# SqueezeAILab/KVQuant

Hardware: NVIDIA H100
Metric: decode tokens/sec @ seqlen 128K (LLaMA-7B, bs1) (higher is better)
Workload: dtype f32

## Files before the change

kvquant_b200/csrc/kvq_kscore.cu:

```cuda
#include "kvq_kscore.cuh"
#include <cuda_fp16.h>
#include <stdlib.h>

namespace kvq {

template <int BITS> struct KCfg {
  static constexpr int N = 1 << BITS;
  static constexpr int W = Layout<BITS>::kWords;
  static constexpr int G = (BITS == 2) ? 16 : 128 / N;
  static constexpr int kThreads = 512;
  static constexpr int TT = kThreads;
  static constexpr int NRW = (BITS == 3) ? 4 : 2;
  static constexpr int D = (BITS == 4) ? 8 : 4;
};

__device__ __forceinline__ void cp_async4(uint32_t smem_dst, const void* gsrc, uint64_t pol, int pred) {
  asm volatile("{ .reg .pred p; setp.ne.s32 p, %3, 0;"
               " @p cp.async.ca.shared.global.L2::cache_hint [%0], [%1], 4, %2; }"
               ::"r"(smem_dst), "l"(gsrc), "l"(pol), "r"(pred) : "memory");
}
__device__ __forceinline__ void cp_async_commit() { asm volatile("cp.async.commit_group;" ::: "memory"); }
template <int N> __device__ __forceinline__ void cp_async_wait() { asm volatile("cp.async.wait_group %0;" ::"n"(N) : "memory"); }
__device__ __forceinline__ uint32_t lds_u32(uint32_t addr) {
  uint32_t v;
  asm volatile("ld.shared.u32 %0, [%1];" : "=r"(v) : "r"(addr));
  return v;
}

template <int BITS> __device__ __forceinline__ int chunk_word_row(int a, int i) {
  if constexpr (BITS == 4) { return i == 0 ? a : a + 8; }
  else if constexpr (BITS == 2) { return i == 0 ? (a >> 1) : 4 + (a >> 1); }
  else {
    const int first = (24 * (a & 3)) >> 5;
    const int w = (i & 1) ? min(first + 1, 2) : first;
    return 3 * ((a >> 2) + ((i >> 1) ? 2 : 0)) + w;
  }
}

template <int BITS>
__device__ __forceinline__ void k_item(const uint32_t* __restrict__ w, const int a, const uint32_t base,
                                       const float2* __restrict__ cs, float2& acc) {
  constexpr int N = 1 << BITS;
  constexpr int HI = kHalf * N * 8;
  if constexpr (BITS == 4) {
    const uint32_t e0 = (w[0] << 3) & 0x78787878u, o0 = (w[0] >> 1) & 0x78787878u;
    const uint32_t e1 = (w[1] << 3) & 0x78787878u, o1 = (w[1] >> 1) & 0x78787878u;
    static_for<0, 8>([&](auto ik) {
      constexpr int k = decltype(ik)::v;
      ffma2(acc, cs[k], lds_f2<k * N * 8>(__byte_perm((k & 1) ? o0 : e0, base, 0x7650 | (k >> 1))));
      ffma2(acc, cs[k], lds_f2<k * N * 8 + HI>(__byte_perm((k & 1) ? o1 : e1, base, 0x7650 | (k >> 1))));
    });
  } else if constexpr (BITS == 2) {
    const int sh = 16 * (a & 1);
    const uint32_t x0 = w[0] >> sh, x1 = w[1] >> sh;
    const uint32_t m00 = (x0 << 3) & 0x1818u, m01 = (x0 << 1) & 0x1818u, m02 = (x0 >> 1) & 0x1818u, m03 = (x0 >> 3) & 0x1818u;
    const uint32_t m10 = (x1 << 3) & 0x1818u, m11 = (x1 << 1) & 0x1818u, m12 = (x1 >> 1) & 0x1818u, m13 = (x1 >> 3) & 0x1818u;
    static_for<0, 8>([&](auto ik) {
      constexpr int k = decltype(ik)::v;
      const uint32_t s0 = (k & 3) == 0 ? m00 : ((k & 3) == 1 ? m01 : ((k & 3) == 2 ? m02 : m03));
      const uint32_t s1 = (k & 3) == 0 ? m10 : ((k & 3) == 1 ? m11 : ((k & 3) == 2 ? m12 : m13));
      ffma2(acc, cs[k], lds_f2<k * N * 8>(__byte_perm(s0, base, 0x7650 | (k >> 2))));
      ffma2(acc, cs[k], lds_f2<k * N * 8 + HI>(__byte_perm(s1, base, 0x7650 | (k >> 2))));
    });
  } else {
    const int sh = (24 * (a & 3)) & 31;
    const uint32_t x0 = __funnelshift_r(w[0], w[1], sh), x1 = __funnelshift_r(w[2], w[3], sh);
    static_for<0, 8>([&](auto ik) {
      constexpr int k = decltype(ik)::v;
      const uint32_t a0 = ((k == 0 ? (x0 << 3) : (x0 >> (3 * k - 3))) & 0x38u) | base;
      const uint32_t a1 = ((k == 0 ? (x1 << 3) : (x1 >> (3 * k - 3))) & 0x38u) | base;
      ffma2(acc, cs[k], lds_f2<k * N * 8>(a0));
      ffma2(acc, cs[k], lds_f2<k * N * 8 + HI>(a1));
    });
  }
}

template <int BITS, bool FULL>
__global__ void __launch_bounds__(KCfg<BITS>::kThreads, 1) k_scores_kernel(const KParams p) {
  using C = KCfg<BITS>;
  constexpr int N = C::N, W = C::W, G = C::G, TT = C::TT, NRW = C::NRW;
  constexpr int PD = (BITS == 4) ? 8 : 4;
  extern __shared__ unsigned char smem_raw[];
  unsigned char* smem = smem_raw + ((256u - (smem_u32(smem_raw) & 255u)) & 255u);
  float2* s_tab = reinterpret_cast<float2*>(smem);
  float* s_q = reinterpret_cast<float*>(s_tab + G * kHeadDim * N);

  const int tid = threadIdx.x;
  const uint64_t pol_stream = policy_evict_first(), pol_keep = policy_evict_last();
  const int h0 = blockIdx.y * G;
  const int nh = FULL ? G : min(G, p.H - h0);

  for (int i = tid; i < nh * kHeadDim; i += C::kThreads) s_q[i] = p.q[(int64_t)h0 * kHeadDim + i];
  __syncthreads();
  for (int i = tid; i < G * kHeadDim * N; i += C::kThreads) {
    float2 e = make_float2(0.f, 0.f);
    if (i < nh * kHeadDim * N) {
      const int hc = i / N;
      const int c = hc & (kHeadDim - 1);
      const float l = p.lut[((int64_t)h0 * kHeadDim) * N + i];
      const float qa = s_q[hc];
      const float qb = s_q[hc ^ kHalf];
      e = make_float2(l * qa, (c < kHalf) ? (l * qb) : -(l * qb));
    }
    s_tab[i] = e;
  }
  __syncthreads();
  const uint32_t tab0 = smem_u32(s_tab);

  const int64_t L_eff = k_eff_len(p);
  const int64_t range = k_eff_range(p, L_eff);
  const int64_t t_begin = (int64_t)blockIdx.x * range;
  const int64_t t_limit = min(L_eff, t_begin + range);
  if (t_begin >= t_limit) return;
  const uint32_t pitch = (uint32_t)p.Lmax * 4u;
  const unsigned char* cb0 = reinterpret_cast<const unsigned char*>(p.cache + (int64_t)h0 * W * p.Lmax);

  const unsigned char* src_cur = cb0 + (t_begin + tid) * 4;
  bool ok_cur = (t_begin + tid) < t_limit;

  uint32_t wq[PD][NRW];
#pragma unroll
  for (int d = 0; d < PD; ++d)
#pragma unroll
    for (int i = 0; i < NRW; ++i) wq[d][i] = 0;
  auto fetch = [&](uint32_t* dst, const unsigned char* base, bool ok, int a, int hl) {
    if (ok && (FULL || hl < nh)) {
#pragma unroll
      for (int i = 0; i < NRW; ++i)
        dst[i] = ld_stream_u32(reinterpret_cast<const uint32_t*>(
                                   base + (uint64_t)(uint32_t)(hl * W + chunk_word_row<BITS>(a, i)) * pitch), pol_stream);
    }
  };
  auto load_cs = [&](float2* dst, const int64_t t, int a) {
    if (t < t_limit) {
      const float2* rp = p.rope + (t + p.pos_offset) + (int64_t)(8 * a) * p.rope_npos;
#pragma unroll
      for (int k = 0; k < 8; ++k) dst[k] = ld_keep_f2(rp + (int64_t)k * p.rope_npos, pol_keep);
    }
  };

  static_for<0, PD>([&](auto id) { constexpr int d = decltype(id)::v; fetch(wq[d], src_cur, ok_cur, 0, d); });
  float2 cs[8], csn[8];
#pragma unroll
  for (int k = 0; k < 8; ++k) { cs[k] = make_float2(0.f, 0.f); csn[k] = make_float2(0.f, 0.f); }
  load_cs(cs, t_begin + tid, 0);

  for (int64_t tb = t_begin; tb < t_limit; tb += TT) {
    const int64_t t = tb + tid;
    const bool live = t < t_limit;
    const unsigned char* src_nxt = src_cur + TT * 4;
    const bool ok_nxt = (t + TT) < t_limit;
    if (tb + (tid & ~31) < t_limit) {
    float2 acc[G];
#pragma unroll
    for (int g = 0; g < G; ++g) acc[g] = make_float2(0.f, 0.f);

    for (int a = 0; a < 8; ++a) {
      load_cs(csn, a == 7 ? t + TT : t, (a + 1) & 7);
      const unsigned char* src_w = (a == 7) ? src_nxt : src_cur;
      const bool ok_w = (a == 7) ? ok_nxt : ok_cur;
      const int a_w = (a + 1) & 7;
      static_for<0, G>([&](auto ig) {
        constexpr int hl = decltype(ig)::v;
        uint32_t w[NRW];
#pragma unroll
        for (int i = 0; i < NRW; ++i) w[i] = wq[hl % PD][i];
        if constexpr (hl + PD < G) fetch(wq[hl % PD], src_cur, ok_cur, a, hl + PD);
        else fetch(wq[hl % PD], src_w, ok_w, a_w, hl + PD - G);
        k_item<BITS>(w, a, tab0 + (uint32_t)hl * (kHeadDim * N * 8) + (uint32_t)a * (8 * N * 8), cs, acc[hl]);
      });
#pragma unroll
      for (int k = 0; k < 8; ++k) cs[k] = csn[k];
    }

    float old[G];
#pragma unroll
    for (int hl = 0; hl < G; ++hl) {
      old[hl] = 0.f;
      if (p.accumulate && live && hl < nh) old[hl] = p.out[(int64_t)(h0 + hl) * p.out_stride + t];
    }
    if (p.opart != nullptr && live) {
      const float4* src = reinterpret_cast<const float4*>(p.opart + t * p.opart_stride + h0);
#pragma unroll
      for (int i = 0; i < G / 4; ++i) {
        const float4 v = __ldcg(src + i);
        old[4 * i] += v.x; old[4 * i + 1] += v.y; old[4 * i + 2] += v.z; old[4 * i + 3] += v.w;
      }
    }
#pragma unroll
    for (int hl = 0; hl < G; ++hl) {
      if (hl < nh) {
        const float s = ((acc[hl].x + acc[hl].y) + old[hl]) * p.scale;
        if (live) p.out[(int64_t)(h0 + hl) * p.out_stride + t] = s;
        if (p.gmax != nullptr) {
          const float m = warp_max(live ? s : -INFINITY);
          if ((tid & 31) == 0 && m > -INFINITY) atomic_max_float(p.gmax + h0 + hl, m);
        }
      }
    }
    }
    src_cur = src_nxt;
    ok_cur = ok_nxt;
  }
}

constexpr int kMaxConstHeads = 48;
__constant__ float4 c_qrot[kMaxConstHeads * kHalf];

template <int BITS> struct KKCfg {
  static constexpr int N = 1 << BITS;
  static constexpr int W = Layout<BITS>::kWords;
  static constexpr int CS = (N * 4 < 32) ? 32 : N * 4;
  static constexpr int G = (BITS == 4) ? 16 : 32;
  static constexpr int kThreads = 512;
  static constexpr int TT = kThreads;
  static constexpr int NRW = (BITS == 3) ? 4 : 2;
  static constexpr int D = 4;
};

template <int IMM>
__device__ __forceinline__ float lds_f1(uint32_t addr) {
  float v;
  asm("ld.shared.f32 %0, [%1+%2];" : "=f"(v) : "r"(addr), "n"(IMM));
  return v;
}
__device__ __forceinline__ float2 fmul2(const float2 a, const float2 b) {
  return make_float2(__fmul_rn(a.x, b.x), __fmul_rn(a.y, b.y));
}

template <int BITS>
__device__ __forceinline__ void kk_item(const uint32_t* __restrict__ w, const int a, const uint32_t base, const int hq,
                                        const float2* __restrict__ cs, float2& acc) {
  using C = KKCfg<BITS>;
  constexpr int CS = C::CS;
  constexpr int HI = kHalf * CS;
  uint32_t alo[8], ahi[8];
  if constexpr (BITS == 4) {
    const uint32_t e0 = (w[0] << 2) & 0x3C3C3C3Cu, o0 = (w[0] >> 2) & 0x3C3C3C3Cu;
    const uint32_t e1 = (w[1] << 2) & 0x3C3C3C3Cu, o1 = (w[1] >> 2) & 0x3C3C3C3Cu;
    static_for<0, 8>([&](auto ik) {
      constexpr int k = decltype(ik)::v;
      alo[k] = __byte_perm((k & 1) ? o0 : e0, base, 0x7650 | (k >> 1));
      ahi[k] = __byte_perm((k & 1) ? o1 : e1, base, 0x7650 | (k >> 1));
    });
  } else if constexpr (BITS == 2) {
    const int sh = 16 * (a & 1);
    const uint32_t x0 = w[0] >> sh, x1 = w[1] >> sh;
    const uint32_t m00 = (x0 << 2) & 0x0C0Cu, m01 = x0 & 0x0C0Cu, m02 = (x0 >> 2) & 0x0C0Cu, m03 = (x0 >> 4) & 0x0C0Cu;
    const uint32_t m10 = (x1 << 2) & 0x0C0Cu, m11 = x1 & 0x0C0Cu, m12 = (x1 >> 2) & 0x0C0Cu, m13 = (x1 >> 4) & 0x0C0Cu;
    static_for<0, 8>([&](auto ik) {
      constexpr int k = decltype(ik)::v;
      const uint32_t s0 = (k & 3) == 0 ? m00 : ((k & 3) == 1 ? m01 : ((k & 3) == 2 ? m02 : m03));
      const uint32_t s1 = (k & 3) == 0 ? m10 : ((k & 3) == 1 ? m11 : ((k & 3) == 2 ? m12 : m13));
      alo[k] = __byte_perm(s0, base, 0x7650 | (k >> 2));
      ahi[k] = __byte_perm(s1, base, 0x7650 | (k >> 2));
    });
  } else {
    const int sh = (24 * (a & 3)) & 31;
    const uint32_t x0 = __funnelshift_r(w[0], w[1], sh), x1 = __funnelshift_r(w[2], w[3], sh);
    static_for<0, 8>([&](auto ik) {
      constexpr int k = decltype(ik)::v;
      alo[k] = ((3 * k >= 2 ? (x0 >> (3 * k - 2)) : (x0 << (2 - 3 * k))) & 0x1Cu) | base;
      ahi[k] = ((3 * k >= 2 ? (x1 >> (3 * k - 2)) : (x1 << (2 - 3 * k))) & 0x1Cu) | base;
    });
  }
  static_for<0, 8>([&](auto ik) {
    constexpr int k = decltype(ik)::v;
    const float2 x = make_float2(lds_f1<k * CS>(alo[k]), lds_f1<k * CS + HI>(ahi[k]));
    const float4 qr = c_qrot[hq * kHalf + 8 * a + k];
    const float2 kap = [&] {
      const float2 t = fmul2(make_float2(cs[k].y, cs[k].y), make_float2(qr.z, qr.w));
      float2 r = t;
      ffma2(r, make_float2(cs[k].x, cs[k].x), make_float2(qr.x, qr.y));
      return r;
    }();
    ffma2(acc, x, kap);
  });
}

template <int BITS>
__global__ void __launch_bounds__(KKCfg<BITS>::kThreads, 1) k_scores_kappa_kernel(const KParams p) {
  using C = KKCfg<BITS>;
  constexpr int N = C::N, W = C::W, G = C::G, TT = C::TT, NRW = C::NRW, D = C::D, CS = C::CS;
  extern __shared__ unsigned char smem_raw[];
  unsigned char* smem = smem_raw + ((256u - (smem_u32(smem_raw) & 255u)) & 255u);
  unsigned char* s_tab = smem;
  uint32_t* s_ring = reinterpret_cast<uint32_t*>(smem + (size_t)G * kHeadDim * CS);

  const int tid = threadIdx.x;
  const uint64_t pol_stream = policy_evict_first(), pol_keep = policy_evict_last();
  const int h0 = blockIdx.y * G;
  const int nh = min(G, p.H - h0);

  for (int i = tid; i < nh * kHeadDim * N; i += C::kThreads) {
    const int hc = i / N, code = i - hc * N;
    *reinterpret_cast<float*>(s_tab + (size_t)hc * CS + code * 4) = p.lut[((int64_t)h0 * kHeadDim) * N + i];
  }
  __syncthreads();
  const uint32_t tab0 = smem_u32(s_tab);
  const uint32_t ring0 = smem_u32(s_ring) + tid * 4;

  const int64_t tile_first = (int64_t)blockIdx.x * p.tiles_per_cta;
  const int64_t tile_end = min(tile_first + p.tiles_per_cta, (p.L + TT - 1) / TT);
  const int64_t t_limit = min(p.L, tile_end * TT);
  const uint32_t* cbase = p.cache + (int64_t)h0 * W * p.Lmax;
  const uint32_t pitch = (uint32_t)p.Lmax * 4u;
  const unsigned char* cb0 = reinterpret_cast<const unsigned char*>(cbase);
  int64_t t_cur = tile_first * TT + tid;
  auto prefetch = [&](int nxt, int a, int hl, int slot) {
    const int64_t t = t_cur + (nxt ? TT : 0);
    const int ok = (t < t_limit) && (hl < nh);
    const unsigned char* src = cb0 + t * 4;
#pragma unroll
    for (int i = 0; i < NRW; ++i)
      cp_async4(ring0 + (uint32_t)(slot * NRW + i) * (TT * 4),
                src + (uint64_t)(uint32_t)(hl * W + chunk_word_row<BITS>(a, i)) * pitch, pol_stream, ok);
    cp_async_commit();
  };
  auto load_cs = [&](float2* dst, int64_t tile, int a) {
    const int64_t t = tile * TT + tid;
    if (t < t_limit) {
      const float2* rp = p.rope + (t + p.pos_offset) + (int64_t)(8 * a) * p.rope_npos;
#pragma unroll
      for (int k = 0; k < 8; ++k) dst[k] = ld_keep_f2(rp + (int64_t)k * p.rope_npos, pol_keep);
    }
  };

  static_for<0, D>([&](auto id) {
    constexpr int d = decltype(id)::v;
    prefetch((d / G) / 8, (d / G) % 8, d % G, d % D);
  });
  float2 cs[8], csn[8];
#pragma unroll
  for (int k = 0; k < 8; ++k) { cs[k] = make_float2(0.f, 0.f); csn[k] = make_float2(0.f, 0.f); }
  load_cs(cs, tile_first, 0);

  for (int64_t tile = tile_first; tile < tile_end; ++tile) {
    const int64_t t = tile * TT + tid;
    t_cur = t;
    const bool live = t < p.L;
    float2 acc[G];
#pragma unroll
    for (int g = 0; g < G; ++g) acc[g] = make_float2(0.f, 0.f);

    for (int a = 0; a < 8; ++a) {
      load_cs(csn, a == 7 ? tile + 1 : tile, (a + 1) & 7);
      static_for<0, G>([&](auto ig) {
        constexpr int hl = decltype(ig)::v;
        cp_async_wait<D - 1>();
        uint32_t w[NRW];
        constexpr int slot = hl % D;
#pragma unroll
        for (int i = 0; i < NRW; ++i) w[i] = lds_u32(ring0 + (uint32_t)(slot * NRW + i) * (TT * 4));
        {
          constexpr int hn = (hl + D) % G;
          constexpr int wrap = (hl + D) / G;
          const int an = a + wrap;
          prefetch(an >> 3, an & 7, hn, slot);
        }
        if (hl < nh)
          kk_item<BITS>(w, a, tab0 + (uint32_t)hl * (kHeadDim * CS) + (uint32_t)a * (8 * CS), h0 + hl, cs, acc[hl]);
      });
#pragma unroll
      for (int k = 0; k < 8; ++k) cs[k] = csn[k];
    }

#pragma unroll
    for (int hl = 0; hl < G; ++hl) {
      if (hl < nh) {
        float s = acc[hl].x + acc[hl].y;
        if (live) {
          float* o = p.out + (int64_t)(h0 + hl) * p.out_stride + t;
          if (p.accumulate) s += *o;
          s *= p.scale;
          *o = s;
        }
        if (p.gmax != nullptr) {
          const float m = warp_max(live ? s : -INFINITY);
          if ((tid & 31) == 0 && m > -INFINITY) atomic_max_float(p.gmax + h0 + hl, m);
        }
      }
    }
  }
  cp_async_wait<0>();
}

__global__ void k_qrot_prep_kernel(const float* __restrict__ q, float4* __restrict__ scratch, int H) {
  const int i = blockIdx.x * blockDim.x + threadIdx.x;
  if (i >= H * kHalf) return;
  const int h = i / kHalf, j = i - h * kHalf;
  const float a = q[h * kHeadDim + j], b = q[h * kHeadDim + j + kHalf];
  scratch[i] = make_float4(a, b, b, -a);
}

static float4* g_qrot_scratch[32] = {nullptr};

static int upload_qrot(const float* q, int H, cudaStream_t st) {
  int dev = 0;
  cudaGetDevice(&dev);
  if (dev < 0 || dev >= 32) return KVQ_E_UNSUPPORTED;
  if (!g_qrot_scratch[dev]) {
    cudaError_t e = cudaMalloc(&g_qrot_scratch[dev], sizeof(float4) * kMaxConstHeads * kHalf);
    if (e != cudaSuccess) return (int)e;
  }
  k_qrot_prep_kernel<<<(H * kHalf + 255) / 256, 256, 0, st>>>(q, g_qrot_scratch[dev], H);
  KVQ_LAUNCH_CHECK();
  cudaError_t e = cudaMemcpyToSymbolAsync(c_qrot, g_qrot_scratch[dev], sizeof(float4) * H * kHalf, 0,
                                          cudaMemcpyDeviceToDevice, st);
  return e == cudaSuccess ? 0 : (int)e;
}

template <int BITS>
static int launch_k_kappa(const KParams& p, cudaStream_t st) {
  using C = KKCfg<BITS>;
  const size_t smem = 256 + (size_t)C::G * kHeadDim * C::CS + (size_t)C::D * C::NRW * C::TT * 4;
  static PerDeviceOnce attr_once;
  bool& attr_done = attr_once.cur();
  if (!attr_done) {
    cudaError_t e = cudaFuncSetAttribute(k_scores_kappa_kernel<BITS>, cudaFuncAttributeMaxDynamicSharedMemorySize, (int)smem);
    if (e != cudaSuccess) return (int)e;
    attr_done = true;
  }
  int rc = upload_qrot(p.q, p.H, st);
  if (rc != 0) return rc;
  const int n_groups = (p.H + C::G - 1) / C::G;
  const int64_t n_tiles = (p.L + C::TT - 1) / C::TT;
  int dev = 0, sms = 132;
  cudaGetDevice(&dev);
  cudaDeviceGetAttribute(&sms, cudaDevAttrMultiProcessorCount, dev);
  const int64_t max_splits = sms / n_groups > 0 ? sms / n_groups : 1;
  KParams q = p;
  q.tiles_per_cta = (int)((n_tiles + max_splits - 1) / max_splits);
  const int64_t splits = (n_tiles + q.tiles_per_cta - 1) / q.tiles_per_cta;
  k_scores_kappa_kernel<BITS><<<dim3((unsigned)splits, (unsigned)n_groups), C::kThreads, smem, st>>>(q);
  KVQ_LAUNCH_CHECK();
  return 0;
}

constexpr int kOutThreads = 256;

__global__ void __launch_bounds__(kOutThreads) k_outlier_kernel(
    const float* __restrict__ q, const float* __restrict__ outliers, const int32_t* __restrict__ outlier_idx,
    float* __restrict__ out, int64_t out_stride, int64_t L, int H, int n_out, const float2* __restrict__ rope,
    int64_t rope_npos, int pos_offset, float scale) {
  const int64_t e = (int64_t)blockIdx.x * kOutThreads + threadIdx.x;
  const int lane = threadIdx.x & 31;
  const int64_t total = L * n_out;
  float contrib = 0.f;
  int64_t key = -1 - lane;
  int64_t t = 0;
  int h = 0;
  if (e < total) {
    t = e / n_out;
    const float v = outliers[e];
    const int col = outlier_idx[e];
    h = col >> 7;
    const int c = col & (kHeadDim - 1);
    key = t * 64 + h;
    if (v != 0.f) {
      const float2 cs = rope[(int64_t)(c & (kHalf - 1)) * rope_npos + t + pos_offset];
      const float sign = (c < kHalf) ? 1.f : -1.f;
      float dot = v * cs.x * __ldg(q + col);
      dot += sign * v * cs.y * __ldg(q + (col ^ kHalf));
      contrib = dot * scale;
    }
  }
#pragma unroll
  for (int o = 1; o < 32; o <<= 1) {
    const float v2 = __shfl_down_sync(0xffffffffu, contrib, o);
    const int64_t k2 = __shfl_down_sync(0xffffffffu, key, o);
    if (lane + o < 32 && k2 == key) contrib += v2;
  }
  const int64_t kprev = __shfl_up_sync(0xffffffffu, key, 1);
  const bool leader = (lane == 0) || (kprev != key);
  if (leader && e < total && contrib != 0.f) atomicAdd(out + (int64_t)h * out_stride + t, contrib);
}

constexpr int kOutPersThreads = 512;
__global__ void __launch_bounds__(kOutPersThreads) k_outlier_pers_kernel(
    const float* __restrict__ q, const float* __restrict__ outliers, const int32_t* __restrict__ outlier_idx,
    float* __restrict__ out, int64_t stride_h, int64_t stride_t, int64_t L, int H, int n_out,
    const float2* __restrict__ rope, int64_t rope_npos, int pos_offset, float scale,
    const int64_t* __restrict__ len_dev, int64_t len_add, const uint32_t* __restrict__ rope_h, float rope_theta) {
  extern __shared__ float2 s_qq[];
  if (len_dev != nullptr) {
    const int64_t l = *len_dev + len_add;
    L = l < 0 ? 0 : (l < L ? l : L);
  }
  const int tid = threadIdx.x, lane = tid & 31;
  for (int i = tid; i < H * kHeadDim; i += kOutPersThreads) s_qq[i] = make_float2(q[i], q[i ^ kHalf]);
  __syncthreads();
  const uint32_t total = (uint32_t)(L * n_out);
  const uint32_t stride = gridDim.x * kOutPersThreads;
  const uint64_t pol_keep = policy_evict_last();
  for (uint32_t base = blockIdx.x * kOutPersThreads + (tid & ~31); base < total; base += stride) {
    const uint32_t e = base + lane;
    float contrib = 0.f;
    int key = -1 - lane;
    uint32_t t = 0;
    int h = 0;
    if (e < total) {
      t = e / (uint32_t)n_out;
      const float v = outliers[e];
      const int col = outlier_idx[e];
      h = col >> 7;
      const int c = col & (kHeadDim - 1);
      key = (int)(t * 64u) + h;
      if (v != 0.f) {
        float2 cs;
        if (rope_theta > 0.f) {
          const int headdim = kHeadDim, headdim2 = headdim / 2;
          const float th = powf(rope_theta, (-2 * __int2float_rd((c & (kHalf - 1)) % headdim2) / __int2float_rd(headdim)));
          const int pos = (int)t + pos_offset;
          cs = make_float2(cosf(th * pos), sinf(th * pos));
        } else if (rope_h != nullptr) {
          uint32_t u;
          asm volatile("ld.global.nc.L2::cache_hint.u32 %0, [%1], %2;" : "=r"(u)
                       : "l"(rope_h + (int64_t)(c & (kHalf - 1)) * rope_npos + t + pos_offset), "l"(pol_keep));
          cs = __half22float2(*reinterpret_cast<const __half2*>(&u));
        } else {
          cs = ld_keep_f2(rope + (int64_t)(c & (kHalf - 1)) * rope_npos + t + pos_offset, pol_keep);
        }
        const float2 qq = s_qq[col];
        const float sign = (c < kHalf) ? 1.f : -1.f;
        float dot = v * cs.x * qq.x;
        dot += sign * v * cs.y * qq.y;
        contrib = dot * scale;
      }
    }
#pragma unroll
    for (int o = 1; o < 32; o <<= 1) {
      const float v2 = __shfl_down_sync(0xffffffffu, contrib, o);
      const int k2 = __shfl_down_sync(0xffffffffu, key, o);
      if (lane + o < 32 && k2 == key) contrib += v2;
    }
    const int kprev = __shfl_up_sync(0xffffffffu, key, 1);
    const bool leader = (lane == 0) || (kprev != key);
    if (leader && e < total && contrib != 0.f) atomicAdd(out + (int64_t)h * stride_h + (int64_t)t * stride_t, contrib);
  }
}

static int k_out_impl_table() {
  static int v = -1;
  if (v < 0) { const char* e = getenv("KVQ_KOUT_IMPL"); v = (e && e[0] == 't') ? 1 : 0; }
  return v;
}

static bool k_out_direct(int64_t n_positions) {
  static int64_t thr = -1;
  if (thr < 0) { const char* e = getenv("KVQ_KOUT_DIRECT_NPOS"); thr = e ? atoll(e) : 64 * 1024; }
  return n_positions > thr;
}

static int launch_k_outliers(const KParams& p, int zero_first, float scale, cudaStream_t st) {
  if (zero_first) {
    cudaError_t e = p.opart != nullptr
        ? cudaMemsetAsync(const_cast<float*>(p.opart), 0, sizeof(float) * (size_t)p.L * (size_t)p.opart_stride, st)
        : cudaMemsetAsync(p.out, 0, sizeof(float) * (size_t)p.H * (size_t)p.out_stride, st);
    if (e != cudaSuccess) return (int)e;
  }
  const int64_t total = p.L * p.n_out;
  const size_t smem = (size_t)p.H * kHeadDim * sizeof(float2);
  if (k_out_impl_table() || smem > 100 * 1024 || total >= ((int64_t)1 << 31) || p.L >= ((int64_t)1 << 25)) {
    if (p.len_dev != nullptr || p.opart != nullptr) return KVQ_E_UNSUPPORTED;
    const unsigned grid = (unsigned)((total + kOutThreads - 1) / kOutThreads);
    k_outlier_kernel<<<grid, kOutThreads, 0, st>>>(p.q, p.outliers, p.outlier_idx, p.out, p.out_stride, p.L, p.H,
                                                   p.n_out, p.rope, p.rope_npos, p.pos_offset, scale);
    KVQ_LAUNCH_CHECK();
    return 0;
  }
  static size_t smem_set_dev[64];
  int dev_idx = 0;
  cudaGetDevice(&dev_idx);
  size_t& smem_set = smem_set_dev[dev_idx & 63];
  if (smem_set == 0) smem_set = 48 * 1024;
  if (smem > smem_set) {
    cudaError_t e = cudaFuncSetAttribute(k_outlier_pers_kernel, cudaFuncAttributeMaxDynamicSharedMemorySize, (int)smem);
    if (e != cudaSuccess) return (int)e;
    smem_set = smem;
  }
  int dev = 0, sms = 132;
  cudaGetDevice(&dev);
  cudaDeviceGetAttribute(&sms, cudaDevAttrMultiProcessorCount, dev);
  const int64_t want = (total + kOutPersThreads - 1) / kOutPersThreads;
  const int per_sm = smem > 56 * 1024 ? 2 : 4;
  const unsigned grid = (unsigned)(want < (int64_t)sms * per_sm ? want : (int64_t)sms * per_sm);
  float* dst = p.opart != nullptr ? const_cast<float*>(p.opart) : p.out;
  const int64_t sh = p.opart != nullptr ? 1 : p.out_stride, stt = p.opart != nullptr ? p.opart_stride : 1;
  k_outlier_pers_kernel<<<grid, kOutPersThreads, smem, st>>>(p.q, p.outliers, p.outlier_idx, dst, sh, stt, p.L,
                                                             p.H, p.n_out, p.rope, p.rope_npos, p.pos_offset, scale,
                                                             p.len_dev, p.len_add, p.rope_h,
                                                             k_out_direct(p.L + p.pos_offset) ? p.theta : 0.f);
  KVQ_LAUNCH_CHECK();
  return 0;
}

__global__ void rope_table_kernel(float2* __restrict__ out, float rope_theta, int64_t n_pos) {
  const int j = blockIdx.y;
  const int headdim = kHeadDim;
  const int headdim2 = headdim / 2;
  const float theta = powf(rope_theta, (-2 * __int2float_rd(j % headdim2) / __int2float_rd(headdim)));
  for (int64_t pos64 = (int64_t)blockIdx.x * blockDim.x + threadIdx.x; pos64 < n_pos; pos64 += (int64_t)gridDim.x * blockDim.x) {
    const int pos = (int)pos64;
    const float c = cosf(theta * pos);
    const float s = sinf(theta * pos);
    out[(int64_t)j * n_pos + pos64] = make_float2(c, s);
  }
}

template <int BITS>
static int launch_k_scores(const KParams& p, cudaStream_t st) {
  using C = KCfg<BITS>;
  const size_t smem = 256 + (size_t)C::G * kHeadDim * C::N * sizeof(float2) + (size_t)C::G * kHeadDim * 4;
  static PerDeviceOnce attr_once;
  bool& attr_done = attr_once.cur();
  if (!attr_done) {
    cudaError_t e = cudaFuncSetAttribute(k_scores_kernel<BITS, true>, cudaFuncAttributeMaxDynamicSharedMemorySize, (int)smem);
    if (e != cudaSuccess) return (int)e;
    e = cudaFuncSetAttribute(k_scores_kernel<BITS, false>, cudaFuncAttributeMaxDynamicSharedMemorySize, (int)smem);
    if (e != cudaSuccess) return (int)e;
    attr_done = true;
  }
  const int n_groups = (p.H + C::G - 1) / C::G;
  int dev = 0, sms = 132;
  cudaGetDevice(&dev);
  cudaDeviceGetAttribute(&sms, cudaDevAttrMultiProcessorCount, dev);
  const int64_t max_splits = sms / n_groups > 0 ? sms / n_groups : 1;
  KParams q = p;
  q.range = k_token_range(p.L, max_splits);
  const int64_t splits = (p.L + q.range - 1) / q.range;
  const dim3 grid((unsigned)splits, (unsigned)n_groups);
  if (p.H % C::G == 0) k_scores_kernel<BITS, true><<<grid, C::kThreads, smem, st>>>(q);
  else k_scores_kernel<BITS, false><<<grid, C::kThreads, smem, st>>>(q);
  KVQ_LAUNCH_CHECK();
  return 0;
}

static int k_impl() {
  static int v = -1;
  if (v < 0) {
    const char* e = getenv("KVQ_K_IMPL");
    v = !e ? 0 : (e[0] == 'g' ? 1 : (e[0] == 'p' ? 2 : (e[0] == 'k' ? 3 : 0)));
  }
  return v;
}

int k_scores_dispatch(int bits, const KParams& p, cudaStream_t st) {
  const int impl = p.len_dev != nullptr ? 0 : k_impl();
  if (impl == 0 && bits == 3) return k_scores3_dispatch(p, st);
  if (impl == 2 && (bits == 4 || bits == 3)) return k_pair_dispatch(bits, p, st);
  if (impl == 3 && p.H <= kMaxConstHeads) {
    switch (bits) {
      case 4: return launch_k_kappa<4>(p, st);
      case 3: return launch_k_kappa<3>(p, st);
      case 2: return launch_k_kappa<2>(p, st);
      default: return KVQ_E_BITS;
    }
  }
  switch (bits) {
    case 4: return launch_k_scores<4>(p, st);
    case 3: return launch_k_scores<3>(p, st);
    case 2: return launch_k_scores<2>(p, st);
    default: return KVQ_E_BITS;
  }
}

int k_scores_fused(int bits, const float* q, const int32_t* cache, float* scores, int64_t score_stride,
                   const float* lut, const float* outliers, const int32_t* outlier_idx, int n_out, int H,
                   int64_t Lmax, int64_t L, const float* rope, int64_t rope_npos, float theta, int pos_offset,
                   float* gmax, float scale, const int64_t* len_dev, int64_t len_add, float* opart, int opart_stride,
                   cudaStream_t st) {
  KParams p{};
  p.len_dev = len_dev; p.len_add = len_add;
  p.q = q; p.cache = reinterpret_cast<const uint32_t*>(cache); p.out = scores; p.lut = lut;
  p.outliers = outliers; p.outlier_idx = outlier_idx; p.rope = reinterpret_cast<const float2*>(rope);
  p.gmax = gmax; p.Lmax = Lmax; p.L = L; p.out_stride = score_stride; p.rope_npos = rope_npos;
  p.H = H; p.n_out = n_out; p.pos_offset = pos_offset; p.scale = scale; p.accumulate = 0; p.theta = theta;
  if (outliers != nullptr) {
    const bool tm = opart != nullptr && !k_out_impl_table() && k_impl() == 0;
    if (tm) { p.opart = opart; p.opart_stride = opart_stride; }
    const int rc = launch_k_outliers(p, 1, 1.f, st);
    if (rc != 0) return rc;
    if (!tm) p.accumulate = 1;
  }
  return k_scores_dispatch(bits, p, st);
}

int k_scores_fused_fast(int bits, const float* q, const int32_t* cache, float* scores, int64_t score_stride,
                        const float* lut, const float* outliers, const int32_t* outlier_idx, int n_out, int H,
                        int64_t Lmax, int64_t L, const float* rope, const void* rope_half, int64_t rope_npos, float theta,
                        int pos_offset, float* gmax, float scale, const int64_t* len_dev, int64_t len_add, void* qtab,
                        cudaStream_t st) {
  static int64_t kBlock = 0;
  if (kBlock == 0) {
    const char* e = getenv("KVQ_K_BLOCK");
    kBlock = e ? (atoll(e) + 31) / 32 * 32 : ((int64_t)1 << 40);
    if (kBlock < 32) kBlock = (int64_t)1 << 40;
  }
  int run_prep = 1;
  for (int64_t t0 = 0; t0 < L; t0 += kBlock) {
    const int64_t Lb = (L - t0 > kBlock + kBlock / 2) ? kBlock : (L - t0);
    int accumulate = 0;
    if (outliers != nullptr) {
      KParams p{};
      p.len_dev = len_dev; p.len_add = len_add - t0;
      p.q = q; p.out = scores + t0; p.outliers = outliers + t0 * n_out; p.outlier_idx = outlier_idx + t0 * n_out;
      p.rope = reinterpret_cast<const float2*>(rope); p.rope_h = static_cast<const uint32_t*>(rope_half);
      p.Lmax = Lmax; p.L = Lb; p.out_stride = score_stride; p.rope_npos = rope_npos;
      p.H = H; p.n_out = n_out; p.pos_offset = pos_offset + (int)t0; p.theta = theta;
      cudaError_t e = cudaMemset2DAsync(scores + t0, sizeof(float) * (size_t)score_stride, 0, sizeof(float) * (size_t)Lb, (size_t)H, st);
      if (e != cudaSuccess) return (int)e;
      const int rc = launch_k_outliers(p, 0, 1.f, st);
      if (rc != 0) return rc;
      accumulate = 1;
    }
    const int rc = (rope_half == nullptr)
        ? k_ratio_dispatch(bits, q, cache, scores, score_stride, lut, H, Lmax, Lb, rope, rope_npos, pos_offset, gmax, scale,
                           accumulate, len_dev, len_add, qtab, t0, run_prep, st)
        : k_fast_dispatch(bits, q, cache, scores, score_stride, lut, H, Lmax, Lb, rope_half, rope_npos, pos_offset, gmax,
                          scale, accumulate, len_dev, len_add, qtab, t0, run_prep, st);
    if (rc != 0) return rc;
    run_prep = 0;
    if (Lb != kBlock) break;
  }
  return 0;
}

}

using namespace kvq;

extern "C" {

int kvq_rope_table_build(float* rope_cos_sin, float theta, int64_t n_pos, void* stream) {
  if (!rope_cos_sin) return KVQ_E_NULL;
  if (n_pos <= 0 || n_pos > (int64_t)1 << 30) return KVQ_E_SHAPE;
  const dim3 grid((unsigned)((n_pos + 255) / 256 > 4096 ? 4096 : (n_pos + 255) / 256), kHalf);
  rope_table_kernel<<<grid, 256, 0, static_cast<cudaStream_t>(stream)>>>(reinterpret_cast<float2*>(rope_cos_sin), theta, n_pos);
  KVQ_LAUNCH_CHECK();
  return 0;
}

int kvq_k_matvec(int bits, const float* q, const int32_t* cache, float* mul, const float* lut, int B, int H,
                 int64_t Lmax, int64_t L, const float* outliers, const int32_t* outlier_idx, int n_out,
                 const float* rope_cos_sin, int64_t rope_npos, float theta, int pos_offset, void* stream) {
  if (!q || !cache || !mul || !lut || !rope_cos_sin) return KVQ_E_NULL;
  if (B <= 0 || H <= 0 || L < 0 || L > Lmax || pos_offset < 0 || Lmax >= ((int64_t)1 << 30)) return KVQ_E_SHAPE;
  if ((outliers == nullptr) != (outlier_idx == nullptr)) return KVQ_E_NULL;
  if (outliers && (B != 1 || n_out <= 0)) return KVQ_E_SHAPE;
  if (outliers && H > 64) return KVQ_E_SHAPE;
  if (rope_npos < L + pos_offset) return KVQ_E_SHAPE;
  if (L == 0) return 0;
  for (int b = 0; b < B; ++b) {
    KParams p{};
    p.q = q + (int64_t)b * H * kHeadDim;
    p.cache = reinterpret_cast<const uint32_t*>(cache);
    p.out = mul + (int64_t)b * H * L;
    p.lut = lut;
    p.outliers = outliers;
    p.outlier_idx = outlier_idx;
    p.rope = reinterpret_cast<const float2*>(rope_cos_sin);
    p.gmax = nullptr;
    p.Lmax = Lmax; p.L = L; p.out_stride = L; p.rope_npos = rope_npos;
    p.H = H; p.n_out = n_out; p.pos_offset = pos_offset;
    p.scale = 1.f; p.accumulate = 1; p.theta = theta;
    if (outliers != nullptr) {
      const int rc0 = launch_k_outliers(p, 0, 1.f, static_cast<cudaStream_t>(stream));
      if (rc0 != 0) return rc0;
    }
    const int rc = k_scores_dispatch(bits, p, static_cast<cudaStream_t>(stream));
    if (rc != 0) return rc;
  }
  return 0;
}

}
```

Measured before the change: 45.21.

## Replace memset plus outlier scatter with warp-tiled outlier score kernel

Outlier key contributions are now computed by a new kernel in which each warp owns a tile of 8 tokens. Contributions for the same token and head are reduced inside the warp by a segmented shuffle and accumulated in a per-warp shared-memory tile, which is then written densely to the score buffer. This removes the separate 2D memset and the scattered global atomic-style accumulation of the old persistent outlier kernel. In exchange it adds shared-memory use per block and caps H at 64.

```diff
diff --git a/kvquant_b200/csrc/kvq_kscore.cu b/kvquant_b200/csrc/kvq_kscore.cu
--- a/kvquant_b200/csrc/kvq_kscore.cu
+++ b/kvquant_b200/csrc/kvq_kscore.cu
@@ -595,6 +595,122 @@
   return 0;
 }
 
+constexpr int kOutTileThreads = 512;
+constexpr int kOutTileTok = 8;
+__global__ void __launch_bounds__(kOutTileThreads, 3) k_outlier_tile_kernel(
+    const float* __restrict__ q, const float* __restrict__ outliers, const int32_t* __restrict__ outlier_idx,
+    float* __restrict__ out, int64_t out_stride, int64_t L, int H, int n_out, const float2* __restrict__ rope,
+    const uint32_t* __restrict__ rope_h, int64_t rope_npos, int pos_offset, const int64_t* __restrict__ len_dev,
+    int64_t len_add, float rope_theta) {
+  constexpr int kWarps = kOutTileThreads / 32;
+  extern __shared__ float2 s_qq[];
+  float* s_th = reinterpret_cast<float*>(s_qq + H * kHeadDim);
+  const int tid = threadIdx.x, lane = tid & 31, warp = tid >> 5;
+  float* s_tile = s_th + kHalf + warp * H * kOutTileTok;
+  if (len_dev != nullptr) {
+    const int64_t l = *len_dev + len_add;
+    L = l < 0 ? 0 : (l < L ? l : L);
+  }
+  for (int i = tid; i < H * kHeadDim; i += kOutTileThreads) s_qq[i] = make_float2(q[i], q[i ^ kHalf]);
+  if (tid < kHalf) {
+    const int headdim = kHeadDim, headdim2 = headdim / 2;
+    s_th[tid] = powf(rope_theta, (-2 * __int2float_rd(tid % headdim2) / __int2float_rd(headdim)));
+  }
+  for (int i = lane; i < H * kOutTileTok; i += 32) s_tile[i] = 0.f;
+  __syncthreads();
+  const uint64_t pol_keep = policy_evict_last();
+  const int64_t n_tiles = (L + kOutTileTok - 1) / kOutTileTok;
+  for (int64_t tile = (int64_t)blockIdx.x * kWarps + warp; tile < n_tiles; tile += (int64_t)gridDim.x * kWarps) {
+    const int64_t tok0 = tile * kOutTileTok;
+    const int ntok = (int)(L - tok0 < kOutTileTok ? L - tok0 : kOutTileTok);
+    const int64_t base = (tok0 * n_out) & ~(int64_t)31;
+    const uint32_t e_lo = (uint32_t)(tok0 * n_out - base), e_hi = e_lo + (uint32_t)(ntok * n_out);
+    const float* ov = outliers + base;
+    const int32_t* oi = outlier_idx + base;
+    for (uint32_t e = lane; e - lane < e_hi; e += 32) {
+      const bool live = e >= e_lo && e < e_hi;
+      float contrib = 0.f;
+      int key = -1 - lane;
+      int tl = 0, h = 0;
+      if (live) {
+        tl = (int)((e - e_lo) / (uint32_t)n_out);
+        const float v = __ldcs(ov + e);
+        const int col = __ldcs(oi + e);
+        h = col >> 7;
+        const int c = col & (kHeadDim - 1);
+        key = tl * 64 + h;
+        if (v != 0.f) {
+          float2 cs;
+          const int j = c & (kHalf - 1);
+          const int pos = (int)(tok0 + tl) + pos_offset;
+          if (rope_theta > 0.f) {
+            const float x = s_th[j] * pos;
+            cs = x <= 105615.f ? make_float2(cosf(x), sinf(x)) : ld_keep_f2(rope + (int64_t)j * rope_npos + pos, pol_keep);
+          } else if (rope_h != nullptr) {
+            uint32_t w;
+            asm volatile("ld.global.nc.L2::cache_hint.u32 %0, [%1], %2;" : "=r"(w)
+                         : "l"(rope_h + (int64_t)j * rope_npos + pos), "l"(pol_keep));
+            cs = __half22float2(*reinterpret_cast<const __half2*>(&w));
+          } else {
+            cs = ld_keep_f2(rope + (int64_t)j * rope_npos + pos, pol_keep);
+          }
+          const float2 qq = s_qq[col];
+          const float sign = (c < kHalf) ? 1.f : -1.f;
+          float dot = v * cs.x * qq.x;
+          dot += sign * v * cs.y * qq.y;
+          contrib = dot;
+        }
+      }
+#pragma unroll
+      for (int o = 1; o < 32; o <<= 1) {
+        const float v2 = __shfl_down_sync(0xffffffffu, contrib, o);
+        const int k2 = __shfl_down_sync(0xffffffffu, key, o);
+        if (lane + o < 32 && k2 == key) contrib += v2;
+      }
+      const int kprev = __shfl_up_sync(0xffffffffu, key, 1);
+      const bool leader = (lane == 0) || (kprev != key);
+      if (leader && live && contrib != 0.f) s_tile[h * kOutTileTok + tl] += contrib;
+      __syncwarp();
+    }
+    for (int i = lane; i < H * kOutTileTok; i += 32) {
+      const int h = i / kOutTileTok, tl = i % kOutTileTok;
+      if (tl < ntok) out[(int64_t)h * out_stride + tok0 + tl] = s_tile[i];
+      s_tile[i] = 0.f;
+    }
+    __syncwarp();
+  }
+}
+
+int num_sms_cached();
+
+static int launch_k_outlier_tiles(const float* q, const float* outliers, const int32_t* outlier_idx, float* out,
+                                  int64_t out_stride, int64_t L, int H, int n_out, const float2* rope,
+                                  const uint32_t* rope_h, int64_t rope_npos, int pos_offset, float theta,
+                                  const int64_t* len_dev, int64_t len_add, cudaStream_t st) {
+  if (H > 64 || n_out <= 0 || (int64_t)kOutTileTok * n_out >= ((int64_t)1 << 31)) return KVQ_E_SHAPE;
+  const size_t smem = (size_t)H * kHeadDim * sizeof(float2) + kHalf * sizeof(float) +
+                      (size_t)(kOutTileThreads / 32) * H * kOutTileTok * sizeof(float);
+  static size_t smem_set_dev[64];
+  int dev = 0;
+  cudaGetDevice(&dev);
+  size_t& smem_set = smem_set_dev[dev & 63];
+  if (smem_set == 0) smem_set = 48 * 1024;
+  if (smem > smem_set) {
+    cudaError_t e = cudaFuncSetAttribute(k_outlier_tile_kernel, cudaFuncAttributeMaxDynamicSharedMemorySize, (int)smem);
+    if (e != cudaSuccess) return (int)e;
+    smem_set = smem;
+  }
+  const int64_t tiles = (L + kOutTileTok - 1) / kOutTileTok;
+  const int64_t want = (tiles + kOutTileThreads / 32 - 1) / (kOutTileThreads / 32);
+  const int64_t cap = (int64_t)num_sms_cached() * 3;
+  const unsigned grid = (unsigned)(want < cap ? (want > 0 ? want : 1) : cap);
+  k_outlier_tile_kernel<<<grid, kOutTileThreads, smem, st>>>(q, outliers, outlier_idx, out, out_stride, L, H, n_out,
+                                                             rope, rope_h, rope_npos, pos_offset, len_dev, len_add,
+                                                             k_out_direct(L + pos_offset) ? theta : 0.f);
+  KVQ_LAUNCH_CHECK();
+  return 0;
+}
+
 __global__ void rope_table_kernel(float2* __restrict__ out, float rope_theta, int64_t n_pos) {
   const int j = blockIdx.y;
   const int headdim = kHeadDim;
@@ -702,15 +818,10 @@
     const int64_t Lb = (L - t0 > kBlock + kBlock / 2) ? kBlock : (L - t0);
     int accumulate = 0;
     if (outliers != nullptr) {
-      KParams p{};
-      p.len_dev = len_dev; p.len_add = len_add - t0;
-      p.q = q; p.out = scores + t0; p.outliers = outliers + t0 * n_out; p.outlier_idx = outlier_idx + t0 * n_out;
-      p.rope = reinterpret_cast<const float2*>(rope); p.rope_h = static_cast<const uint32_t*>(rope_half);
-      p.Lmax = Lmax; p.L = Lb; p.out_stride = score_stride; p.rope_npos = rope_npos;
-      p.H = H; p.n_out = n_out; p.pos_offset = pos_offset + (int)t0; p.theta = theta;
-      cudaError_t e = cudaMemset2DAsync(scores + t0, sizeof(float) * (size_t)score_stride, 0, sizeof(float) * (size_t)Lb, (size_t)H, st);
-      if (e != cudaSuccess) return (int)e;
-      const int rc = launch_k_outliers(p, 0, 1.f, st);
+      const int rc = launch_k_outlier_tiles(q, outliers + t0 * n_out, outlier_idx + t0 * n_out, scores + t0, score_stride,
+                                            Lb, H, n_out, reinterpret_cast<const float2*>(rope),
+                                            static_cast<const uint32_t*>(rope_half), rope_npos, pos_offset + (int)t0,
+                                            theta, len_dev, len_add - t0, st);
       if (rc != 0) return rc;
       accumulate = 1;
     }
```

Result: faster. 46.61 (median of 6 runs) (+3.1%).
